# Deeptanshu-sankhwar/horizonml

Hardware: AMD Instinct MI355X
Metric: images/sec (higher is better)
Workload: dtype bf16; 1 GPU; model=resnet18_cifar10, global_batch=64, image=3x32x32, parallelism=dp1, optimizer=adam, exec=graph, comm=none

## Files before the change

### horizonml_amd/engine/flat.py

```python
from __future__ import annotations

from typing import List

import torch
import torch.nn as nn

from .. import ops as _ops
from ..models.layers import ConvBNAct, DepthwiseConvBNAct, Linear


SEG_CHUNK = 4096


class SegmentTable:

    def __init__(self, sizes, decay, adapt, device, chunk: int = SEG_CHUNK):
        sizes = [int(n) for n in sizes]
        if not sizes or min(sizes) < 1 or chunk < 1:
            raise ValueError("segments must be non-empty")
        if not len(sizes) == len(decay) == len(adapt):
            raise ValueError("one decay and one adapt flag per segment")
        if sum(sizes) >= 2 ** 31:
            raise ValueError("segment offsets are int32")
        chunks, meta, bounds = [], [], [0]
# ... 24 lines not shown
        self.lars, self.eta = bool(lars), float(eta)
        self.seg_mul = t.static_mul(self.wd)
        self.dynamic = self.max_norm > 0 or self.lars
        if self.dynamic:
            dev = mgr.master.device
            self.partials = torch.zeros(t.nchunks, 2, device=dev)
            self.seg_norms = torch.zeros(t.nseg, 2, device=dev)
            self.norm_out = torch.zeros(2, device=dev)

    def reduce(self, ext, mgr, grad_bf16, grad_scale):
        if self.dynamic:
            ext.seg_norms(mgr.master, mgr.grad, self.table.chunks,
                          self.table.seg_meta, self.partials, self.seg_norms,
                          self.seg_mul, self.norm_out, self.wd, self.max_norm,
                          self.lars, self.eta, grad_bf16, grad_scale)

    def last_grad_norm(self) -> float:
        if not self.dynamic:
            raise RuntimeError("the gradient norm is only computed with "
                               "clip_grad_norm > 0 or lars")
        return float(self.norm_out[0].cpu())


def _seg_state(mgr, wd, no_decay_1d, max_norm, lars=False, eta=1e-3):
    if max_norm < 0 or eta <= 0:
        raise ValueError("clip_grad_norm must be >= 0 and lars_eta > 0")
    if not (no_decay_1d or max_norm > 0 or lars):
        return None
    return _SegState(mgr, wd, no_decay_1d, max_norm, lars, eta)


class FlatParamManager:
    def __init__(self, model: nn.Module, device: torch.device):
        self._seg_tables = {}
        _ops.extension().set_wgrad_defer(True)
        params = [p for p in model.parameters() if p.requires_grad]
        total = sum(p.numel() for p in params)
        self.params = params
        self.numel = total
        self.master = torch.zeros(total, device=device)
        self.grad = torch.zeros(total, device=device)
        self.shadow = torch.zeros(total, device=device, dtype=torch.bfloat16)
        self.slices = {}
        off = 0
        for p in params:
            n = p.numel()
            with torch.no_grad():
                self.master[off:off + n].copy_(p.data.flatten())
            p.data = self.master[off:off + n].view(p.shape)
            p.grad = self.grad[off:off + n].view(p.shape)
            self.slices[id(p)] = (off, n)
            off += n
        with torch.no_grad():
            self.shadow.copy_(self.master)

        convs = []
        for m in model.modules():
            if isinstance(m, (ConvBNAct, Linear, DepthwiseConvBNAct)):
                woff, wn = self.slices[id(m.weight)]
                m.weight_bf16 = self.shadow[woff:woff + wn].view(
                    m.weight.shape)
                m._managed = True
                if isinstance(m, ConvBNAct):
                    convs.append((m, woff, wn))
        stats_total = sum(2 * m.out_ch for m, _, _ in convs)
        self.stats_arena = torch.zeros(max(1, stats_total), device=device)
        soff = 0
        for m, _, _ in convs:
            m._stats_buf = self.stats_arena[soff:soff + 2 * m.out_ch]
            soff += 2 * m.out_ch

        self.meta = None
        self.max_elem = 1
        if _ops.extension().dgrad_krsc_enabled():
            self.rsck = torch.zeros(0, device=device, dtype=torch.bfloat16)
            for m, _, _ in convs:
                if hasattr(m, "_w_rsck"):
                    del m._w_rsck
            return
        rsck_total = sum(wn for _, _, wn in convs)
        self.rsck = torch.zeros(rsck_total, device=device,
                                dtype=torch.bfloat16)
        meta: List[List[int]] = []
        doff = 0
        self.max_elem = 1
        for m, woff, wn in convs:
            K, R, S, C = m.weight.shape
# ... 3 lines not shown
            self.max_elem = max(self.max_elem, wn)
        self.meta = (torch.tensor(meta, dtype=torch.int32, device=device)
                     if meta else None)
        self.refresh_rsck()

    def refresh_rsck(self):
        if self.meta is not None:
            _ops.extension().permute_krsc_rsck(self.shadow, self.rsck,
                                               self.meta, self.max_elem)

    def zero_grad(self):
        self.grad.zero_()

    def segment_table(self, no_decay_1d: bool = False) -> SegmentTable:
        key = bool(no_decay_1d)
        if key not in self._seg_tables:
            one_d = [p.ndim <= 1 for p in self.params]
            self._seg_tables[key] = SegmentTable(
                [p.numel() for p in self.params],
                [not (key and d) for d in one_d], [not d for d in one_d],
                self.master.device)
        return self._seg_tables[key]


def _sched_buffers(schedule, dev):
    if schedule is None:
        return None, None
    return schedule.table().to(dev), torch.zeros(1, device=dev)


class HorizonAdam:

    def __init__(self, mgr: FlatParamManager, lr: float = 1e-3,
                 betas=(0.9, 0.999), eps: float = 1e-8,
                 weight_decay: float = 0.0, schedule=None,
                 decoupled_wd: bool = False, no_decay_1d: bool = False,
                 clip_grad_norm: float = 0.0):
        self.mgr = mgr
        self.seg = _seg_state(mgr, weight_decay, no_decay_1d, clip_grad_norm)
        self.lr, self.betas, self.eps, self.wd = lr, betas, eps, weight_decay
        self.schedule, self.decoupled = schedule, bool(decoupled_wd)
        dev = mgr.master.device
        self.m = torch.zeros_like(mgr.master)
        self.v = torch.zeros_like(mgr.master)
        self.step_t = torch.zeros(1, device=dev)
        self.lr_table, self.lr_out = _sched_buffers(schedule, dev)

    def step(self, zero_grad: bool = True, grad_bf16=None,
             grad_scale: float = 1.0, probe=None):
        ext = _ops.extension()
        ext.flush_wgrad()
        p0, p1, p2 = probe if probe is not None else (None, None, None)
        if self.seg is not None:
            self.seg.reduce(ext, self.mgr, grad_bf16, grad_scale)
            ext.adam_step_seg(self.mgr.master, self.mgr.grad, self.m, self.v,
                              self.mgr.shadow, self.step_t, self.lr_table,
                              self.lr_out, self.lr, self.betas[0],
                              self.betas[1], self.eps, self.decoupled,
                              zero_grad, self.seg.table.chunks,
                              self.seg.seg_mul, self.mgr.stats_arena,
                              grad_bf16, grad_scale, p0, p1, p2)
        elif self.schedule is None and not self.decoupled:
            ext.adam_step(self.mgr.master, self.mgr.grad, self.m,
                          self.v, self.mgr.shadow, self.step_t,
                          self.lr, self.betas[0], self.betas[1],
                          self.eps, self.wd, zero_grad,
                          self.mgr.stats_arena, grad_bf16,
                          grad_scale, p0, p1, p2)
        else:
            ext.adam_step_sched(self.mgr.master, self.mgr.grad, self.m,
                                self.v, self.mgr.shadow, self.step_t,
                                self.lr_table, self.lr_out, self.lr,
                                self.betas[0], self.betas[1], self.eps,
                                self.wd, self.decoupled, zero_grad,
                                self.mgr.stats_arena, grad_bf16, grad_scale,
                                p0, p1, p2)
        self.mgr.refresh_rsck()

    def current_lr(self) -> float:
        if self.lr_out is None:
            return float(self.lr)
        return float(self.lr_out.cpu())

    def last_grad_norm(self) -> float:
        if self.seg is None:
            raise RuntimeError("the gradient norm is only computed with "
                               "clip_grad_norm > 0 or lars")
        return self.seg.last_grad_norm()

    def set_step(self, n: int):
        self.step_t.fill_(float(n))

    def state_dict(self):
        return {"kind": "horizon_adam", "lr": self.lr, "betas": self.betas,
                "eps": self.eps, "weight_decay": self.wd,
                "m": self.m.detach().cpu(), "v": self.v.detach().cpu(),
                "step_t": self.step_t.detach().cpu()}

    def load_state_dict(self, state):
        if state.get("kind") != "horizon_adam":
            raise ValueError("checkpoint optimizer state is not HorizonAdam")
        with torch.no_grad():
            self.m.copy_(state["m"].to(self.m.device))
            self.v.copy_(state["v"].to(self.v.device))
            self.step_t.copy_(state["step_t"].to(self.step_t.device))


class HorizonSGD:

    def __init__(self, mgr: FlatParamManager, lr: float = 0.1,
                 momentum: float = 0.9, weight_decay: float = 0.0,
                 schedule=None, nesterov: bool = False,
                 no_decay_1d: bool = False, clip_grad_norm: float = 0.0,
                 lars: bool = False, lars_eta: float = 1e-3):
        if nesterov and not momentum > 0:
            raise ValueError("nesterov needs momentum > 0")
        self.mgr = mgr
        self.seg = _seg_state(mgr, weight_decay, no_decay_1d, clip_grad_norm,
                              lars, lars_eta)
        self.lr, self.mu, self.wd = lr, momentum, weight_decay
        self.schedule, self.nesterov = schedule, bool(nesterov)
        self.mom = (torch.zeros_like(mgr.master) if momentum > 0 else None)
        dev = mgr.master.device
        self.lr_table, self.lr_out = _sched_buffers(schedule, dev)
        self.step_t = (torch.zeros(1, device=dev)
                       if schedule is not None else None)

    def step(self, zero_grad: bool = True, grad_bf16=None,
             grad_scale: float = 1.0, probe=None):
        ext = _ops.extension()
        ext.flush_wgrad()
        p0, p1, p2 = probe if probe is not None else (None, None, None)
        if self.seg is not None:
            self.seg.reduce(ext, self.mgr, grad_bf16, grad_scale)
            ext.sgd_step_seg(self.mgr.master, self.mgr.grad, self.mom,
                             self.mgr.shadow, self.step_t, self.lr_table,
                             self.lr_out, self.lr, self.mu, self.nesterov,
                             zero_grad, self.seg.table.chunks,
                             self.seg.seg_mul, grad_bf16, grad_scale,
                             p0, p1, p2)
        elif self.schedule is None and not self.nesterov:
            ext.sgd_step(self.mgr.master, self.mgr.grad, self.mom,
                         self.mgr.shadow, self.lr, self.mu, self.wd,
                         zero_grad, grad_bf16, grad_scale,
                         p0, p1, p2)
        else:
            ext.sgd_step_sched(self.mgr.master, self.mgr.grad, self.mom,
                               self.mgr.shadow, self.step_t, self.lr_table,
                               self.lr_out, self.lr, self.mu, self.wd,
                               self.nesterov, zero_grad, grad_bf16,
                               grad_scale, p0, p1, p2)
        self.mgr.stats_arena.zero_()
        self.mgr.refresh_rsck()

    def current_lr(self) -> float:
        if self.lr_out is None:
            return float(self.lr)
        return float(self.lr_out.cpu())

    def last_grad_norm(self) -> float:
        if self.seg is None:
            raise RuntimeError("the gradient norm is only computed with "
                               "clip_grad_norm > 0 or lars")
        return self.seg.last_grad_norm()

    def set_step(self, n: int):
        if self.step_t is not None:
            self.step_t.fill_(float(n))

    def state_dict(self):
        state = {"kind": "horizon_sgd", "lr": self.lr, "momentum": self.mu,
                 "weight_decay": self.wd,
                 "mom": (self.mom.detach().cpu()
                         if self.mom is not None else None)}
        if self.step_t is not None:
            state["step_t"] = self.step_t.detach().cpu()
        return state

    def load_state_dict(self, state):
        if state.get("kind") != "horizon_sgd":
            raise ValueError("checkpoint optimizer state is not HorizonSGD")
        if (state.get("mom") is None) != (self.mom is None):
            raise ValueError("momentum buffer mismatch with checkpoint")
        with torch.no_grad():
            if self.mom is not None:
                self.mom.copy_(state["mom"].to(self.mom.device))
            if self.step_t is not None and state.get("step_t") is not None:
                self.step_t.copy_(state["step_t"].to(self.step_t.device))
```

### horizonml_amd/ops/csrc/bind.cpp

```cpp
#include <torch/extension.h>
#include <c10/hip/HIPStream.h>
#include <c10/hip/HIPCachingAllocator.h>

#include <memory>
#include <vector>

#include "launch.h"

namespace {

using torch::Tensor;

hipStream_t cur_stream() { return c10::hip::getCurrentHIPStream().stream(); }

bool g_deterministic = false;
void set_deterministic(bool on) {
  g_deterministic = on;
  set_kernels_deterministic(on ? 1 : 0);
}
bool deterministic_enabled() { return g_deterministic; }

void set_bn_owner(bool on) { set_kernels_bn_owner(on ? 1 : 0); }
bool bn_owner_enabled() { return kernels_bn_owner() != 0; }
std::vector<int64_t> bn_owner_launches() {
  long f = 0, b = 0;
  bn_owner_launch_counts(&f, &b);
  return {(int64_t)f, (int64_t)b};
// ... 9 lines not shown

bool g_tap_clip = env_long("HZ_TAP_CLIP", 1) != 0;
void set_tap_clip(bool on) { g_tap_clip = on; }
bool tap_clip_enabled() { return g_tap_clip; }

std::vector<int64_t> conv_tap_window(int64_t H, int64_t W, int64_t R,
                                     int64_t S, int64_t stride, int64_t pad) {
  TORCH_CHECK(stride >= 1 && pad >= 0 && R >= 1 && S >= 1 &&
                  H + 2 * pad >= R && W + 2 * pad >= S,
              "conv_tap_window: empty output or bad geometry");
  ConvP p{};
  p.H = (int)H;
  p.W = (int)W;
  p.C = 1;
  p.R = p.Rf = (int)R;
  p.S = p.Sf = (int)S;
  p.str = (int)stride;
  p.pad = (int)pad;
  p.Ho = (p.H + 2 * p.pad - p.R) / p.str + 1;
  p.Wo = (p.W + 2 * p.pad - p.S) / p.str + 1;
  p = clip_taps(p);
  return {p.r0, p.s0, p.R, p.S};
}

struct PendingWgrad {
  torch::Tensor x, dconv, dw;
  ConvP p;
};

bool g_wgrad_defer = false;
std::vector<PendingWgrad> g_pending;
torch::Tensor g_wgrad_ws;

void set_wgrad_defer(bool on) { g_wgrad_defer = on; }
bool wgrad_defer_enabled() { return g_wgrad_defer; }
int64_t wgrad_pending() { return (int64_t)g_pending.size(); }

static inline int cdiv_i(long a, long b) { return (int)((a + b - 1) / b); }

void flush_one_group(int lo, int hi);

void flush_wgrad() {
  if (g_pending.empty()) return;
  const int total = (int)g_pending.size();
  int lo = 0;
  while (lo < total) {
// ... 403 lines not shown
  if (has_res) {
    dres = empty_cl_bf16(p.Nb, K, p.Ho, p.Wo, x);
    dres_ptr = dres.data_ptr();
  }
  if (own)
    launch_bn_bwd_owner(dy.data_ptr(), y.data_ptr(), convout.data_ptr(),
                        save_mean.data_ptr<float>(),
                        save_invstd.data_ptr<float>(),
                        gamma.data_ptr<float>(), beta.data_ptr<float>(),
                        sum_dz.data_ptr<float>(), sum_dzx.data_ptr<float>(),
                        dconv.data_ptr(), dres_ptr, (long)p.M, K, mask_mode,
                        own, st);
  else
    launch_bn_bwd_apply(dy.data_ptr(), y.data_ptr(), convout.data_ptr(),
                        save_mean.data_ptr<float>(),
                        save_invstd.data_ptr<float>(),
                        gamma.data_ptr<float>(), beta.data_ptr<float>(),
                        sum_dz.data_ptr<float>(), sum_dzx.data_ptr<float>(),
                        dconv.data_ptr(), dres_ptr, (long)p.M, K, mask_mode,
                        st);

  Tensor dw = direct ? *dw_out
                     : at::zeros({(int64_t)K, R, S, (int64_t)p.C}, fopt);
  if (direct && g_wgrad_defer) {
    g_pending.push_back({x, dconv, dw, p});
  } else {
    int msplit = wgrad_msplit(p);
    Tensor ws;
    float* ws_ptr = nullptr;
    if (msplit > 1) {
      ws = at::empty({(long)msplit * K * p.Kd}, fopt);
      ws_ptr = ws.data_ptr<float>();
    }
    launch_wgrad(x.data_ptr(), dconv.data_ptr(), dw.data_ptr<float>(), ws_ptr,
                 p, (int)g_wgrad_tr, st);
  }

  TORCH_CHECK(need_dx || !fuse_up.has_value(),
              "fuse_up requires need_dx (the fused reduce rides the dx "
              "production)");
  Tensor dx;
  if (need_dx)
    dx = dgrad_dx(dconv, w, w_rsck, p, dx_accum, fuse_up, (int)up_mask_mode,
                  st);
  return {dx, dw, sum_dzx, sum_dz, dres};
}
// ... 535 lines not shown
                  c10::optional<Tensor> probe_sumsq,
                  c10::optional<Tensor> probe_out) {
  check_f32(master, "master");
  check_probe(probe_prev, probe_sumsq, probe_out);
  TORCH_CHECK(grad.numel() == master.numel()
                  && (!mom.has_value() || mom->numel() == master.numel()),
              "grad / mom must match master's size");
  TORCH_CHECK(!nesterov || (mom.has_value() && mu > 0.0),
              "nesterov needs a momentum buffer and momentum > 0");
  SegTable t = seg_table(chunks, seg_mul, master);
  long T = 0;
  const float* table = sched_table(lr_table, master, &T);
  TORCH_CHECK(table == nullptr || step_t.has_value(),
              "lr_table needs the step_t device counter");
  float* out = sched_scalar(lr_out, master, "lr_out");
  float* st = sched_scalar(step_t, master, "step_t");
  launch_sgd_step_seg(master.data_ptr<float>(), grad.data_ptr<float>(),
                      opt_ptr<float>(mom), opt_ptr(shadow), (float)lr,
                      (float)mu, zero_grad ? 1 : 0, opt_ptr(grad_bf16),
                      (float)grad_scale, opt_ptr<float>(probe_prev),
                      opt_ptr<float>(probe_sumsq), opt_ptr<float>(probe_out),
                      st, table, T, out, nesterov ? 1 : 0, t.chunks,
                      t.nchunks, t.seg_mul, cur_stream());
}

void permute_krsc_rsck(Tensor src, Tensor dst, Tensor meta,
                       int64_t max_elem) {
  TORCH_CHECK(meta.scalar_type() == torch::kInt32 && meta.is_cuda());
  launch_permute_krsc_rsck(src.data_ptr(), dst.data_ptr(),
                           meta.data_ptr<int>(), (int)meta.size(0),
                           (int)max_elem, cur_stream());
}

void grad_divergence(Tensor g, Tensor prev, Tensor sumsq, Tensor out,
                     bool skip_first) {
  launch_grad_divergence(g.data_ptr<float>(), prev.data_ptr<float>(),
                         sumsq.data_ptr<float>(), out.data_ptr<float>(),
                         g.numel(), skip_first ? 1 : 0, cur_stream());
}

void bn_reduce_bench(Tensor dy, Tensor y, Tensor x, Tensor mean,
                     Tensor invstd, Tensor gamma, Tensor beta, Tensor sdz,
                     Tensor sdzx, int64_t M, int64_t C, int64_t mask) {
  launch_bnact_bwd_reduce(dy.data_ptr(), y.data_ptr(), x.data_ptr(),
                          mean.data_ptr<float>(), invstd.data_ptr<float>(),
                          gamma.data_ptr<float>(), beta.data_ptr<float>(),
// ... 154 lines not shown
        py::arg("probe_out") = py::none());
  m.def("seg_norms", &seg_norms, py::arg("master"), py::arg("grad"),
        py::arg("chunks"), py::arg("seg_meta"), py::arg("partials"),
        py::arg("seg_norms"), py::arg("seg_mul"), py::arg("norm_out"),
        py::arg("wd"), py::arg("max_norm"), py::arg("lars"), py::arg("eta"),
        py::arg("grad_bf16") = py::none(), py::arg("grad_scale") = 1.0);
  m.def("adam_step_seg", &adam_step_seg, py::arg("master"), py::arg("grad"),
        py::arg("m"), py::arg("v"), py::arg("shadow"), py::arg("step_t"),
        py::arg("lr_table"), py::arg("lr_out"), py::arg("lr"), py::arg("b1"),
        py::arg("b2"), py::arg("eps"), py::arg("decoupled"),
        py::arg("zero_grad"), py::arg("chunks"), py::arg("seg_mul"),
        py::arg("extra_zero") = py::none(), py::arg("grad_bf16") = py::none(),
        py::arg("grad_scale") = 1.0, py::arg("probe_prev") = py::none(),
        py::arg("probe_sumsq") = py::none(),
        py::arg("probe_out") = py::none());
  m.def("sgd_step_seg", &sgd_step_seg, py::arg("master"), py::arg("grad"),
        py::arg("mom"), py::arg("shadow"), py::arg("step_t"),
        py::arg("lr_table"), py::arg("lr_out"), py::arg("lr"), py::arg("mu"),
        py::arg("nesterov"), py::arg("zero_grad"), py::arg("chunks"),
        py::arg("seg_mul"), py::arg("grad_bf16") = py::none(),
        py::arg("grad_scale") = 1.0, py::arg("probe_prev") = py::none(),
        py::arg("probe_sumsq") = py::none(),
        py::arg("probe_out") = py::none());
  m.def("permute_krsc_rsck", &permute_krsc_rsck);
  m.def("grad_divergence", &grad_divergence);
  m.def("normalize_u8", &normalize_u8);
  m.def("augment_normalize_u8", &augment_normalize_u8, py::arg("x"),
        py::arg("state"), py::arg("mean"), py::arg("std"), py::arg("pad"),
        py::arg("flip"), py::arg("params") = py::none());
  m.def("bn_reduce_bench", &bn_reduce_bench);
  m.def("bn_fwd_pair_bench", &bn_fwd_pair_bench);
  m.def("bn_bwd_pair_bench", &bn_bwd_pair_bench);
  m.def("set_bn_owner", &set_bn_owner);
  m.def("bn_owner_enabled", &bn_owner_enabled);
  m.def("bn_owner_launches", &bn_owner_launches);
  m.def("set_deterministic", &set_deterministic);
  m.def("deterministic_enabled", &deterministic_enabled);
  m.def("set_wgrad_defer", &set_wgrad_defer);
  m.def("wgrad_defer_enabled", &wgrad_defer_enabled);
  m.def("wgrad_pending", &wgrad_pending);
  m.def("flush_wgrad", &flush_wgrad);
  m.def("flush_wgrad_range", &flush_wgrad_range);
  m.def("wgrad_only", &wgrad_only);
  m.def("conv_dgrad_only", &conv_dgrad_only);
  m.def("set_dgrad_krsc", &set_dgrad_krsc);
  m.def("dgrad_krsc_enabled", &dgrad_krsc_enabled);
// ... 7 lines not shown
```

### horizonml_amd/ops/csrc/elem_kernels.hip

```cpp
#include <cstdio>

#include "common.h"

union F8 {
  float4 q[2];
  float f[8];
};

DEV F8 load_f8(const float* p) {
  F8 v;
  v.q[0] = *(const float4*)p;
  v.q[1] = *(const float4*)(p + 4);
  return v;
}

template <bool F32SRC, int ACT, bool TRAIN>
__global__ __launch_bounds__(256) void k_bn_apply(
    const void* __restrict__ xv, const bf16* __restrict__ res,
    bf16* __restrict__ y, bf16* __restrict__ convout,
    const float* __restrict__ stats,
    const float* __restrict__ gamma, const float* __restrict__ beta,
    float* __restrict__ running_mean, float* __restrict__ running_var,
    float* __restrict__ save_mean, float* __restrict__ save_invstd,
    long M, int C, float momentum, float eps, int nsplit) {
// ... 1499 lines not shown
    const float* __restrict__ logits, const long* __restrict__ target,
    float* __restrict__ loss, float* __restrict__ dlogits, int B, int NC) {
  ce_body<false>(logits, target, loss, dlogits, B, NC, 0.f,
                 blockIdx.x * blockDim.x + threadIdx.x,
                 gridDim.x * blockDim.x);
}

__global__ __launch_bounds__(256) void k_ce_ls_fwd_bwd_det(
    const float* __restrict__ logits, const long* __restrict__ target,
    float* __restrict__ loss, float* __restrict__ dlogits, int B, int NC,
    float eps) {
  ce_det_body<true>(logits, target, loss, dlogits, B, NC, eps);
}

__global__ __launch_bounds__(256) void k_ce_ls_fwd_bwd(
    const float* __restrict__ logits, const long* __restrict__ target,
    float* __restrict__ loss, float* __restrict__ dlogits, int B, int NC,
    float eps) {
  ce_body<true>(logits, target, loss, dlogits, B, NC, eps,
                blockIdx.x * blockDim.x + threadIdx.x,
                gridDim.x * blockDim.x);
}

template <bool DECOUPLED, bool SEG = false>
__device__ __forceinline__ void adam_body(
    float* __restrict__ master, float* __restrict__ grad,
    float* __restrict__ m, float* __restrict__ v, bf16* __restrict__ shadow,
    const float* __restrict__ step_t, long n, float lr, float b1, float b2,
    float eps, float wd, int zero_grad, float* __restrict__ extra_zero,
    long n_extra, const bf16* __restrict__ gsrc, float gscale,
    float* __restrict__ prev, float* __restrict__ sumsq, long i0,
    long istride, float gmul = 1.f) {
  for (long i = i0; i < n_extra; i += istride) extra_zero[i] = 0.f;
  float t = step_t[0];
  float bc1 = 1.f - __powf(b1, t), bc2 = 1.f - __powf(b2, t);
  float acc = 0.f;
  for (long i = i0; i < n; i += istride) {
    float gl = grad[i];
    float g = gsrc != nullptr ? b2f(gsrc[i]) * gscale : gl;
    if (prev != nullptr) {
      float d = gl - prev[i];
      prev[i] = gl;
      acc += d * d;
    }
    if (SEG && gmul != 1.f) g *= gmul;
    float w = master[i];
    if (DECOUPLED) {
      if (wd != 0.f) w *= 1.f - lr * wd;
    } else {
      if (wd != 0.f) g += wd * w;
    }
    float mi = b1 * m[i] + (1.f - b1) * g;
    float vi = b2 * v[i] + (1.f - b2) * g * g;
    m[i] = mi;
    v[i] = vi;
    w -= lr * (mi / bc1) / (sqrtf(vi / bc2) + eps);
    master[i] = w;
    if (shadow != nullptr) shadow[i] = f2b(w);
    if (zero_grad) grad[i] = 0.f;
  }
  if (prev != nullptr) {
    acc = wave_reduce_sum(acc);
    __shared__ float ws[4];
    if ((threadIdx.x & 63) == 0) ws[threadIdx.x >> 6] = acc;
    __syncthreads();
    if (threadIdx.x == 0)
      atomicAdd(sumsq, ws[0] + ws[1] + ws[2] + ws[3]);
  }
}

template <bool NESTEROV, bool SEG = false>
__device__ __forceinline__ void sgd_body(
    float* __restrict__ master, float* __restrict__ grad,
    float* __restrict__ mom, bf16* __restrict__ shadow, long n, float lr,
    float mu, float wd, int zero_grad, const bf16* __restrict__ gsrc,
    float gscale, float* __restrict__ prev, float* __restrict__ sumsq,
    long i0, long istride, float gmul = 1.f) {
  float acc = 0.f;
  for (long i = i0; i < n; i += istride) {
    float gl = grad[i];
    float g = gsrc != nullptr ? b2f(gsrc[i]) * gscale : gl;
    if (prev != nullptr) {
      float d = gl - prev[i];
      prev[i] = gl;
      acc += d * d;
    }
    if (SEG && gmul != 1.f) g *= gmul;
    float w = master[i];
    if (wd != 0.f) g += wd * w;
    float u = (mom != nullptr) ? (mu * mom[i] + g) : g;
    if (mom != nullptr) mom[i] = u;
    if (NESTEROV)
      w -= lr * (g + mu * u);
    else
      w -= lr * u;
    master[i] = w;
    if (shadow != nullptr) shadow[i] = f2b(w);
    if (zero_grad) grad[i] = 0.f;
  }
  if (prev != nullptr) {
    acc = wave_reduce_sum(acc);
    __shared__ float ws[4];
// ... 229 lines not shown
__global__ __launch_bounds__(256) void k_adam_step_seg(
    float* __restrict__ master, float* __restrict__ grad,
    float* __restrict__ m, float* __restrict__ v, bf16* __restrict__ shadow,
    const float* __restrict__ step_t, float lr, float b1, float b2,
    float eps, int zero_grad, float* __restrict__ extra_zero, long n_extra,
    const bf16* __restrict__ gsrc, float gscale, float* __restrict__ prev,
    float* __restrict__ sumsq, const float* __restrict__ lr_table, long T,
    float* __restrict__ lr_out, const int* __restrict__ chunks,
    const float* __restrict__ seg_mul) {
  lr = sched_lr(step_t, lr_table, T, lr, lr_out);
  for (long i = (long)blockIdx.x * 256 + threadIdx.x; i < n_extra;
       i += (long)gridDim.x * 256)
    extra_zero[i] = 0.f;
  const int c = blockIdx.x;
  const int s = chunks[c * 3];
  const long start = chunks[c * 3 + 1];
  const long end = start + chunks[c * 3 + 2];
  adam_body<DECOUPLED, true>(master, grad, m, v, shadow, step_t, end, lr, b1,
                             b2, eps, seg_mul[2 * s + 1], zero_grad, nullptr,
                             0, gsrc, gscale, prev, sumsq,
                             start + threadIdx.x, 256, seg_mul[2 * s]);
}

__global__ __launch_bounds__(256) void k_permute_krsc_rsck(
    const bf16* __restrict__ src, bf16* __restrict__ dst,
    const int* __restrict__ meta, int nconv) {
  __shared__ bf16 tile[32][33];
  const int ci = blockIdx.y;
  if (ci >= nconv) return;
  const int soff = meta[ci * 4 + 0], doff = meta[ci * 4 + 1];
  const int nelem = meta[ci * 4 + 2];
  const int K = meta[ci * 4 + 3] >> 16, C = meta[ci * 4 + 3] & 0xffff;
  const int RS = nelem / (K * C);
  const int ktiles = (K + 31) / 32, ctiles = (C + 31) / 32;
  const int tiles_per_rs = ktiles * ctiles;
  const int total_tiles = RS * tiles_per_rs;
  const int tc = threadIdx.x & 31, tr = threadIdx.x >> 5;
  for (int t = blockIdx.x; t < total_tiles; t += gridDim.x) {
    int rs = t / tiles_per_rs, rem = t % tiles_per_rs;
    int k0 = (rem / ctiles) * 32, c0 = (rem % ctiles) * 32;
    const bf16* s = src + soff + (long)rs * C;
#pragma unroll
    for (int i = 0; i < 4; i++) {
      int ko = k0 + tr + i * 8, c = c0 + tc;
      tile[tr + i * 8][tc] = (ko < K && c < C)
          ? s[(long)ko * RS * C + c] : (bf16)0.f;
// ... 666 lines not shown
  if (decoupled) LA(true); else LA(false);
#undef LA
  if (prev != nullptr)
    k_gdiv_finalize<<<1, 1, 0, st>>>(sumsq, divout, 0);
}

void launch_sgd_step_seg(float* master, float* grad, float* mom, void* shadow,
                         float lr, float mu, int zero_grad, const void* gsrc,
                         float gscale, float* prev, float* sumsq,
                         float* divout, float* step_t, const float* lr_table,
                         long T, float* lr_out, int nesterov,
                         const int* chunks, int nchunks, const float* seg_mul,
                         hipStream_t st) {
  if (lr_table != nullptr) k_inc_step<<<1, 1, 0, st>>>(step_t);
#define LS(N) k_sgd_step_seg<N><<<nchunks, 256, 0, st>>>( \
    master, grad, mom, (bf16*)shadow, lr, mu, zero_grad, (const bf16*)gsrc, \
    gscale, prev, sumsq, step_t, lr_table, T, lr_out, chunks, seg_mul)
  if (nesterov) LS(true); else LS(false);
#undef LS
  if (prev != nullptr)
    k_gdiv_finalize<<<1, 1, 0, st>>>(sumsq, divout, 0);
}

void launch_permute_krsc_rsck(const void* src, void* dst, const int* meta,
                              int nconv, int max_elem, hipStream_t st) {
  dim3 grid(gsz((long)max_elem, 1024), nconv);
  k_permute_krsc_rsck<<<grid, 256, 0, st>>>((const bf16*)src, (bf16*)dst,
                                            meta, nconv);
}

void launch_grad_divergence(const float* g, float* prev, float* sumsq,
                            float* out, long n, int skip_first,
                            hipStream_t st) {
  k_gdiv_partial<<<gsz(n >> 2), 256, 0, st>>>(g, prev, sumsq, n);
  k_gdiv_finalize<<<1, 1, 0, st>>>(sumsq, out, skip_first);
}

void launch_normalize_u8(const void* x, void* y, long total, int C, long HW,
                         float mean, float std, hipStream_t st) {
  k_normalize_u8<<<gsz(total), 256, 0, st>>>((const unsigned char*)x,
                                             (bf16*)y, total, C, HW, mean,
                                             std);
}

void launch_augment_normalize_u8(const void* x, void* y, void* state,
                                 const int* params, long N, int C, int H,
// ... 17 lines not shown
```

### horizonml_amd/ops/csrc/launch.h

```cpp
#pragma once
#include <hip/hip_runtime_api.h>

#include <cstdlib>
#include <type_traits>

struct ConvP {
  int Nb, H, W, C, K;
  int Ho, Wo, R, S;
  int str, pad;
  int M, Kd;
  int r0, s0, Rf, Sf;
};

struct MagicP {
  unsigned m[4];
  int s[4];
  unsigned d[4];
};

constexpr int WG_MAX_TASKS = 20;

struct WgradTask {
  const void* X;
  const void* Dz;
// ... 81 lines not shown
        last = r;
        break;
      }
    }
  *lo = last < 0 ? 0 : first;
  *n = last < 0 ? 0 : last - first + 1;
}

inline ConvP clip_taps(ConvP p) {
  int r0, rn, s0, sn;
  tap_range(p.H, p.Ho, p.Rf, p.str, p.pad, &r0, &rn);
  tap_range(p.W, p.Wo, p.Sf, p.str, p.pad, &s0, &sn);
  if (rn <= 0 || sn <= 0) return p;
  p.r0 = r0;
  p.s0 = s0;
  p.R = rn;
  p.S = sn;
  p.Kd = rn * sn * p.C;
  return p;
}

inline bool taps_clipped(const ConvP& p) {
  return p.R != p.Rf || p.S != p.Sf;
}

inline long env_long(const char* name, long dflt) {
  const char* e = getenv(name);
  return e ? atol(e) : dflt;
}

extern "C" {

int conv_fwd_splitk(ConvP p);
int conv_dgrad_splitk(ConvP p);
void launch_conv_fwd(const void* x, const void* w, void* y, float* stats,
                     ConvP p, hipStream_t st);
void launch_conv_fwd_splitk(const void* x, const void* w, float* ws, ConvP p,
                            int splitk, hipStream_t st);
void launch_conv_dgrad(const void* dz, const void* w, void* dx, float* ws,
                       int splitk, ConvP p, int accum, int w_layout,
                       hipStream_t st);
void launch_gemm_bf16(const void* a, const void* b, void* c, int M, int N,
                      int K, hipStream_t st);
int wgrad_msplit(ConvP p);
void launch_wgrad(const void* x, const void* dz, float* dw, float* ws,
                  ConvP p, int tr, hipStream_t st);
// ... 110 lines not shown
                        const float* lr_table, long T, float* lr_out,
                        int nesterov, hipStream_t st);
void launch_seg_norms(const float* master, const float* grad,
                      const void* gsrc, float gscale, const int* chunks,
                      int nchunks, const int* seg_meta, int nseg,
                      float* partials, float* seg_norms, float* seg_mul,
                      float* norm_out, float wd, float max_norm, int lars,
                      float eta, hipStream_t st);
void launch_adam_step_seg(float* master, float* grad, float* m, float* v,
                          void* shadow, float* step_t, float lr, float b1,
                          float b2, float eps, int zero_grad,
                          float* extra_zero, long n_extra, const void* gsrc,
                          float gscale, float* prev, float* sumsq,
                          float* divout, const float* lr_table, long T,
                          float* lr_out, int decoupled, const int* chunks,
                          int nchunks, const float* seg_mul, hipStream_t st);
void launch_sgd_step_seg(float* master, float* grad, float* mom, void* shadow,
                         float lr, float mu, int zero_grad, const void* gsrc,
                         float gscale, float* prev, float* sumsq,
                         float* divout, float* step_t, const float* lr_table,
                         long T, float* lr_out, int nesterov,
                         const int* chunks, int nchunks, const float* seg_mul,
                         hipStream_t st);

void launch_permute_krsc_rsck(const void* src, void* dst, const int* meta,
                              int nconv, int max_elem, hipStream_t st);
void launch_grad_divergence(const float* g, float* prev, float* sumsq,
                            float* out, long n, int skip_first,
                            hipStream_t st);
void launch_normalize_u8(const void* x, void* y, long total, int C, long HW,
                         float mean, float std, hipStream_t st);
void launch_augment_normalize_u8(const void* x, void* y, void* state,
                                 const int* params, long N, int C, int H,
                                 int W, int pad, int flip, float mean,
                                 float std, hipStream_t st);

}
```

Baseline: 71560 images/sec.

## Skip optimizer updates on structurally dead conv filter taps via a live-chunk table

Records, per weight-gradient buffer, the range of filter taps that can ever receive gradient given the conv geometry. From that it builds a strided chunk table covering only live weight elements. New Adam and SGD kernels walk this table, so the optimizer skips weights whose gradient is structurally zero. Buffers with nonzero values in dead taps are demoted to full updates. The cost is host-side table building, registry bookkeeping and strided access. The table is not built during graph capture.

```diff
diff --git a/horizonml_amd/engine/flat.py b/horizonml_amd/engine/flat.py
--- a/horizonml_amd/engine/flat.py
+++ b/horizonml_amd/engine/flat.py
@@ -70,6 +70,77 @@
         return float(self.norm_out[0].cpu())
 
 
+LIVE_CHUNK = 4096
+
+
+def build_live_chunks(numel, windows, chunk: int = LIVE_CHUNK):
+    numel, chunk = int(numel), int(chunk)
+    if numel < 1 or numel >= 2 ** 31 or chunk < 1:
+        raise ValueError("live table offsets are int32")
+    spans, families, cursor, n_dead = [], [], 0, 0
+    for off, K, Rf, Sf, C, r0, R, s0, S in sorted(
+            tuple(int(x) for x in w) for w in windows):
+        kdf = Rf * Sf * C
+        if min(K, Rf, Sf, C, R, S) < 1 or min(r0, s0) < 0 \
+                or r0 + R > Rf or s0 + S > Sf:
+            raise ValueError("tap window outside its filter")
+        if off < cursor or off + K * kdf > numel:
+            raise ValueError("conv weights overlap or leave the buffer")
+        if R == Rf and S == Sf:
+            continue
+        if off > cursor:
+            spans.append((cursor, off))
+        cursor = off + K * kdf
+        n_dead += K * (Rf * Sf - R * S) * C
+        if S == Sf:
+            families.append((off + r0 * Sf * C, R * Sf * C, kdf, K))
+        else:
+            families += [(off + ((r0 + r) * Sf + s0) * C, S * C, kdf, K)
+                         for r in range(R)]
+    if cursor < numel:
+        spans.append((cursor, numel))
+
+    chunks = []
+
+    def cut(lo, hi):
+        chunks.extend((o, min(chunk, hi - o), 0, 1)
+                      for o in range(lo, hi, chunk))
+
+    for lo, hi in spans:
+        cut(lo, hi)
+    for start, run_len, pitch, nruns in families:
+        if run_len >= chunk or nruns == 1:
+            for r in range(nruns):
+                cut(start + r * pitch, start + r * pitch + run_len)
+            continue
+        group = chunk // run_len
+        chunks.extend((start + r * pitch, run_len, pitch,
+                       min(group, nruns - r))
+                      for r in range(0, nruns, group))
+    for start, run_len, pitch, nruns in chunks:
+        if not (run_len >= 1 and nruns >= 1 and run_len * nruns <= chunk
+                and start >= 0 and pitch >= 0
+                and (nruns == 1 or pitch >= run_len)
+                and start + (nruns - 1) * pitch + run_len <= numel):
+            raise AssertionError("live chunk out of bounds")
+    return chunks, n_dead
+
+
+class _LiveTable:
+
+    def __init__(self):
+        self.version = -1
+        self.bufs = []
+        self.chunks = None
+        self.n_dead = 0
+        self.n_demoted = 0
+        self.nchunks = 0
+
+    def covers(self, bufs):
+        have = {t.data_ptr() for t in self.bufs}
+        return all(t.data_ptr() in have for t in bufs)
+
+
 def _seg_state(mgr, wd, no_decay_1d, max_norm, lars=False, eta=1e-3):
     if max_norm < 0 or eta <= 0:
         raise ValueError("clip_grad_norm must be >= 0 and lars_eta > 0")
@@ -88,6 +159,8 @@
         self.numel = total
         self.master = torch.zeros(total, device=device)
         self.grad = torch.zeros(total, device=device)
+        _ops.extension().tap_window_reset(
+            self.grad.data_ptr(), self.grad.data_ptr() + 4 * total)
         self.shadow = torch.zeros(total, device=device, dtype=torch.bfloat16)
         self.slices = {}
         off = 0
@@ -111,6 +184,9 @@
                 m._managed = True
                 if isinstance(m, ConvBNAct):
                     convs.append((m, woff, wn))
+        self._conv_shapes = {woff: tuple(m.weight.shape)
+                             for m, woff, _ in convs}
+        self._live = _LiveTable()
         stats_total = sum(2 * m.out_ch for m, _, _ in convs)
         self.stats_arena = torch.zeros(max(1, stats_total), device=device)
         soff = 0
@@ -160,6 +236,72 @@
                 self.master.device)
         return self._seg_tables[key]
 
+    def live_windows(self):
+        base, out = self.grad.data_ptr(), []
+        for ptr, K, Rf, Sf, C, r0, R, s0, S in \
+                _ops.extension().tap_window_registry():
+            off, rem = divmod(ptr - base, 4)
+            if rem == 0 and self._conv_shapes.get(off) == (K, Rf, Sf, C):
+                out.append((off, K, Rf, Sf, C, r0, R, s0, S))
+        return sorted(out)
+
+    def invalidate_live_table(self):
+        self._live.version = -1
+
+    def live_table_info(self):
+        lt = self._live
+        state = ("unbuilt" if lt.version < 0
+                 else "none" if lt.chunks is None else "live")
+        return {"state": state, "version": lt.version,
+                "skipped": lt.n_dead if state == "live" else 0,
+                "nchunks": lt.nchunks if state == "live" else 0,
+                "demoted": lt.n_demoted}
+
+    def live_chunks(self, bufs):
+        ext = _ops.extension()
+        if not ext.opt_skip_dead_enabled():
+            return None
+        lt = self._live
+        bufs = [t for t in bufs if t is not None]
+        version = ext.tap_window_version()
+        if lt.version != version or not lt.covers(bufs):
+            if torch.cuda.is_current_stream_capturing():
+                return None
+            have = {t.data_ptr() for t in bufs}
+            bufs += [t for t in lt.bufs if t.data_ptr() not in have]
+            self._build_live_table(version, bufs)
+        return lt.chunks
+
+    def _build_live_table(self, version, bufs):
+        lt = self._live
+        wins = self.live_windows()
+        clipped = [w for w in wins if w[6] * w[8] < w[2] * w[3]]
+        lt.n_demoted = 0
+        if clipped:
+            counts = []
+            for off, K, Rf, Sf, C, r0, R, s0, S in clipped:
+                n, c = K * Rf * Sf * C, 0
+                for t in [self.grad] + bufs:
+                    bits = t[off:off + n].view(
+                        torch.int32 if t.element_size() == 4 else torch.int16
+                    ).view(K, Rf, Sf, C)
+                    c = c + torch.count_nonzero(bits) - torch.count_nonzero(
+                        bits[:, r0:r0 + R, s0:s0 + S])
+                counts.append(c)
+            bad = torch.stack(counts).cpu().tolist()
+            lt.n_demoted = sum(1 for b in bad if b)
+            clipped = [w for w, b in zip(clipped, bad) if not b]
+        chunks, lt.n_dead = build_live_chunks(self.numel, clipped)
+        if lt.n_dead:
+            lt.chunks = torch.tensor(chunks, dtype=torch.int32,
+                                     device=self.master.device)
+            lt.nchunks = len(chunks)
+            with torch.no_grad():
+                self.shadow.copy_(self.master)
+        else:
+            lt.chunks, lt.nchunks = None, 0
+        lt.version, lt.bufs = version, bufs
+
 
 def _sched_buffers(schedule, dev):
     if schedule is None:
@@ -183,12 +325,16 @@
         self.v = torch.zeros_like(mgr.master)
         self.step_t = torch.zeros(1, device=dev)
         self.lr_table, self.lr_out = _sched_buffers(schedule, dev)
+        self._live_stale = False
 
     def step(self, zero_grad: bool = True, grad_bf16=None,
              grad_scale: float = 1.0, probe=None):
         ext = _ops.extension()
         ext.flush_wgrad()
         p0, p1, p2 = probe if probe is not None else (None, None, None)
+        if self._live_stale:
+            self.mgr.invalidate_live_table()
+            self._live_stale = False
         if self.seg is not None:
             self.seg.reduce(ext, self.mgr, grad_bf16, grad_scale)
             ext.adam_step_seg(self.mgr.master, self.mgr.grad, self.m, self.v,
@@ -198,6 +344,14 @@
                               zero_grad, self.seg.table.chunks,
                               self.seg.seg_mul, self.mgr.stats_arena,
                               grad_bf16, grad_scale, p0, p1, p2)
+        elif self.wd == 0 and (live := self.mgr.live_chunks(
+                (self.m, self.v, p0, grad_bf16))) is not None:
+            ext.adam_step_live(self.mgr.master, self.mgr.grad, self.m,
+                               self.v, self.mgr.shadow, self.step_t,
+                               self.lr_table, self.lr_out, self.lr,
+                               self.betas[0], self.betas[1], self.eps,
+                               zero_grad, live, self.mgr.stats_arena,
+                               grad_bf16, grad_scale, p0, p1, p2)
         elif self.schedule is None and not self.decoupled:
             ext.adam_step(self.mgr.master, self.mgr.grad, self.m,
                           self.v, self.mgr.shadow, self.step_t,
@@ -238,6 +392,7 @@
     def load_state_dict(self, state):
         if state.get("kind") != "horizon_adam":
             raise ValueError("checkpoint optimizer state is not HorizonAdam")
+        self._live_stale = True
         with torch.no_grad():
             self.m.copy_(state["m"].to(self.m.device))
             self.v.copy_(state["v"].to(self.v.device))
@@ -263,12 +418,16 @@
         self.lr_table, self.lr_out = _sched_buffers(schedule, dev)
         self.step_t = (torch.zeros(1, device=dev)
                        if schedule is not None else None)
+        self._live_stale = False
 
     def step(self, zero_grad: bool = True, grad_bf16=None,
              grad_scale: float = 1.0, probe=None):
         ext = _ops.extension()
         ext.flush_wgrad()
         p0, p1, p2 = probe if probe is not None else (None, None, None)
+        if self._live_stale:
+            self.mgr.invalidate_live_table()
+            self._live_stale = False
         if self.seg is not None:
             self.seg.reduce(ext, self.mgr, grad_bf16, grad_scale)
             ext.sgd_step_seg(self.mgr.master, self.mgr.grad, self.mom,
@@ -277,6 +436,13 @@
                              zero_grad, self.seg.table.chunks,
                              self.seg.seg_mul, grad_bf16, grad_scale,
                              p0, p1, p2)
+        elif self.wd == 0 and (live := self.mgr.live_chunks(
+                (self.mom, p0, grad_bf16))) is not None:
+            ext.sgd_step_live(self.mgr.master, self.mgr.grad, self.mom,
+                              self.mgr.shadow, self.step_t, self.lr_table,
+                              self.lr_out, self.lr, self.mu, self.nesterov,
+                              zero_grad, live, grad_bf16, grad_scale,
+                              p0, p1, p2)
         elif self.schedule is None and not self.nesterov:
             ext.sgd_step(self.mgr.master, self.mgr.grad, self.mom,
                          self.mgr.shadow, self.lr, self.mu, self.wd,
@@ -320,6 +486,7 @@
             raise ValueError("checkpoint optimizer state is not HorizonSGD")
         if (state.get("mom") is None) != (self.mom is None):
             raise ValueError("momentum buffer mismatch with checkpoint")
+        self._live_stale = True
         with torch.no_grad():
             if self.mom is not None:
                 self.mom.copy_(state["mom"].to(self.mom.device))
diff --git a/horizonml_amd/ops/csrc/bind.cpp b/horizonml_amd/ops/csrc/bind.cpp
--- a/horizonml_amd/ops/csrc/bind.cpp
+++ b/horizonml_amd/ops/csrc/bind.cpp
@@ -2,7 +2,10 @@
 #include <c10/hip/HIPStream.h>
 #include <c10/hip/HIPCachingAllocator.h>
 
+#include <algorithm>
 #include <memory>
+#include <mutex>
+#include <unordered_map>
 #include <vector>
 
 #include "launch.h"
@@ -58,6 +61,73 @@
   p = clip_taps(p);
   return {p.r0, p.s0, p.R, p.S};
 }
+
+struct TapWindow {
+  int K, Rf, Sf, C;
+  int r0, R, s0, S;
+};
+std::mutex g_tapwin_mu;
+std::unordered_map<uintptr_t, TapWindow> g_tapwin;
+int64_t g_tapwin_version = 0;
+
+void record_tap_window(const Tensor& dw, const ConvP& p) {
+  const ConvP g = geometric_taps(p);
+  const uintptr_t key = (uintptr_t)dw.data_ptr();
+  std::lock_guard<std::mutex> lock(g_tapwin_mu);
+  auto it = g_tapwin.find(key);
+  if (it == g_tapwin.end() || it->second.K != g.K || it->second.Rf != g.Rf ||
+      it->second.Sf != g.Sf || it->second.C != g.C) {
+    g_tapwin[key] = {g.K, g.Rf, g.Sf, g.C, g.r0, g.R, g.s0, g.S};
+    g_tapwin_version++;
+    return;
+  }
+  TapWindow& w = it->second;
+  const int r0 = std::min(w.r0, g.r0), s0 = std::min(w.s0, g.s0);
+  const int r1 = std::max(w.r0 + w.R, g.r0 + g.R);
+  const int s1 = std::max(w.s0 + w.S, g.s0 + g.S);
+  if (r0 != w.r0 || s0 != w.s0 || r1 - r0 != w.R || s1 - s0 != w.S) {
+    w.r0 = r0;
+    w.R = r1 - r0;
+    w.s0 = s0;
+    w.S = s1 - s0;
+    g_tapwin_version++;
+  }
+}
+
+std::vector<std::vector<int64_t>> tap_window_registry() {
+  std::lock_guard<std::mutex> lock(g_tapwin_mu);
+  std::vector<std::vector<int64_t>> out;
+  out.reserve(g_tapwin.size());
+  for (const auto& kv : g_tapwin) {
+    const TapWindow& w = kv.second;
+    out.push_back({(int64_t)kv.first, w.K, w.Rf, w.Sf, w.C, w.r0, w.R, w.s0,
+                   w.S});
+  }
+  return out;
+}
+
+int64_t tap_window_version() {
+  std::lock_guard<std::mutex> lock(g_tapwin_mu);
+  return g_tapwin_version;
+}
+
+void tap_window_reset(int64_t lo, int64_t hi) {
+  std::lock_guard<std::mutex> lock(g_tapwin_mu);
+  if (hi <= lo) {
+    g_tapwin.clear();
+  } else {
+    for (auto it = g_tapwin.begin(); it != g_tapwin.end();)
+      if (it->first >= (uintptr_t)lo && it->first < (uintptr_t)hi)
+        it = g_tapwin.erase(it);
+      else
+        ++it;
+  }
+  g_tapwin_version++;
+}
+
+bool g_opt_skip_dead = env_long("HZ_OPT_SKIP_DEAD", 1) != 0;
+void set_opt_skip_dead(bool on) { g_opt_skip_dead = on; }
+bool opt_skip_dead_enabled() { return g_opt_skip_dead; }
 
 struct PendingWgrad {
   torch::Tensor x, dconv, dw;
@@ -507,6 +577,7 @@
 
   Tensor dw = direct ? *dw_out
                      : at::zeros({(int64_t)K, R, S, (int64_t)p.C}, fopt);
+  if (direct) record_tap_window(dw, p);
   if (direct && g_wgrad_defer) {
     g_pending.push_back({x, dconv, dw, p});
   } else {
@@ -1088,6 +1159,86 @@
                       opt_ptr<float>(probe_sumsq), opt_ptr<float>(probe_out),
                       st, table, T, out, nesterov ? 1 : 0, t.chunks,
                       t.nchunks, t.seg_mul, cur_stream());
+}
+
+const int* live_table(const Tensor& live, const Tensor& master,
+                      int* nchunks) {
+  TORCH_CHECK(live.scalar_type() == torch::kInt32 && live.dim() == 2
+                  && live.size(1) == 4 && live.size(0) >= 1
+                  && live.is_contiguous()
+                  && live.device() == master.device()
+                  && (uintptr_t)live.data_ptr() % 16 == 0,
+              "live must be a contiguous, 16-byte aligned int32 [nchunks,4] "
+              "tensor on master's device");
+  *nchunks = (int)live.size(0);
+  return live.data_ptr<int>();
+}
+
+void adam_step_live(Tensor master, Tensor grad, Tensor m, Tensor v,
+                    c10::optional<Tensor> shadow, Tensor step_t,
+                    c10::optional<Tensor> lr_table,
+                    c10::optional<Tensor> lr_out, double lr, double b1,
+                    double b2, double eps, bool zero_grad, Tensor live,
+                    c10::optional<Tensor> extra_zero,
+                    c10::optional<Tensor> grad_bf16, double grad_scale,
+                    c10::optional<Tensor> probe_prev,
+                    c10::optional<Tensor> probe_sumsq,
+                    c10::optional<Tensor> probe_out) {
+  check_f32(master, "master");
+  check_probe(probe_prev, probe_sumsq, probe_out);
+  TORCH_CHECK(grad.numel() == master.numel() && m.numel() == master.numel()
+                  && v.numel() == master.numel(),
+              "grad / m / v must match master's size");
+  int nchunks = 0;
+  const int* chunks = live_table(live, master, &nchunks);
+  long T = 0;
+  const float* table = sched_table(lr_table, master, &T);
+  float* out = sched_scalar(lr_out, master, "lr_out");
+  float* st = sched_scalar(step_t, master, "step_t");
+  launch_adam_step_live(master.data_ptr<float>(), grad.data_ptr<float>(),
+                        m.data_ptr<float>(), v.data_ptr<float>(),
+                        opt_ptr(shadow), st, (float)lr, (float)b1, (float)b2,
+                        (float)eps, zero_grad ? 1 : 0,
+                        opt_ptr<float>(extra_zero),
+                        extra_zero.has_value() ? extra_zero->numel() : 0,
+                        opt_ptr(grad_bf16), (float)grad_scale,
+                        opt_ptr<float>(probe_prev),
+                        opt_ptr<float>(probe_sumsq),
+                        opt_ptr<float>(probe_out), table, T, out, chunks,
+                        nchunks, cur_stream());
+}
+
+void sgd_step_live(Tensor master, Tensor grad, c10::optional<Tensor> mom,
+                   c10::optional<Tensor> shadow, c10::optional<Tensor> step_t,
+                   c10::optional<Tensor> lr_table,
+                   c10::optional<Tensor> lr_out, double lr, double mu,
+                   bool nesterov, bool zero_grad, Tensor live,
+                   c10::optional<Tensor> grad_bf16, double grad_scale,
+                   c10::optional<Tensor> probe_prev,
+                   c10::optional<Tensor> probe_sumsq,
+                   c10::optional<Tensor> probe_out) {
+  check_f32(master, "master");
+  check_probe(probe_prev, probe_sumsq, probe_out);
+  TORCH_CHECK(grad.numel() == master.numel()
+                  && (!mom.has_value() || mom->numel() == master.numel()),
+              "grad / mom must match master's size");
+  TORCH_CHECK(!nesterov || (mom.has_value() && mu > 0.0),
+              "nesterov needs a momentum buffer and momentum > 0");
+  int nchunks = 0;
+  const int* chunks = live_table(live, master, &nchunks);
+  long T = 0;
+  const float* table = sched_table(lr_table, master, &T);
+  TORCH_CHECK(table == nullptr || step_t.has_value(),
+              "lr_table needs the step_t device counter");
+  float* out = sched_scalar(lr_out, master, "lr_out");
+  float* st = sched_scalar(step_t, master, "step_t");
+  launch_sgd_step_live(master.data_ptr<float>(), grad.data_ptr<float>(),
+                       opt_ptr<float>(mom), opt_ptr(shadow), (float)lr,
+                       (float)mu, zero_grad ? 1 : 0, opt_ptr(grad_bf16),
+                       (float)grad_scale, opt_ptr<float>(probe_prev),
+                       opt_ptr<float>(probe_sumsq), opt_ptr<float>(probe_out),
+                       st, table, T, out, nesterov ? 1 : 0, chunks, nchunks,
+                       cur_stream());
 }
 
 void permute_krsc_rsck(Tensor src, Tensor dst, Tensor meta,
@@ -1288,6 +1439,29 @@
         py::arg("grad_scale") = 1.0, py::arg("probe_prev") = py::none(),
         py::arg("probe_sumsq") = py::none(),
         py::arg("probe_out") = py::none());
+  m.def("adam_step_live", &adam_step_live, py::arg("master"),
+        py::arg("grad"), py::arg("m"), py::arg("v"), py::arg("shadow"),
+        py::arg("step_t"), py::arg("lr_table"), py::arg("lr_out"),
+        py::arg("lr"), py::arg("b1"), py::arg("b2"), py::arg("eps"),
+        py::arg("zero_grad"), py::arg("live"),
+        py::arg("extra_zero") = py::none(), py::arg("grad_bf16") = py::none(),
+        py::arg("grad_scale") = 1.0, py::arg("probe_prev") = py::none(),
+        py::arg("probe_sumsq") = py::none(),
+        py::arg("probe_out") = py::none());
+  m.def("sgd_step_live", &sgd_step_live, py::arg("master"), py::arg("grad"),
+        py::arg("mom"), py::arg("shadow"), py::arg("step_t"),
+        py::arg("lr_table"), py::arg("lr_out"), py::arg("lr"), py::arg("mu"),
+        py::arg("nesterov"), py::arg("zero_grad"), py::arg("live"),
+        py::arg("grad_bf16") = py::none(), py::arg("grad_scale") = 1.0,
+        py::arg("probe_prev") = py::none(),
+        py::arg("probe_sumsq") = py::none(),
+        py::arg("probe_out") = py::none());
+  m.def("tap_window_registry", &tap_window_registry);
+  m.def("tap_window_version", &tap_window_version);
+  m.def("tap_window_reset", &tap_window_reset, py::arg("lo") = 0,
+        py::arg("hi") = 0);
+  m.def("set_opt_skip_dead", &set_opt_skip_dead);
+  m.def("opt_skip_dead_enabled", &opt_skip_dead_enabled);
   m.def("permute_krsc_rsck", &permute_krsc_rsck);
   m.def("grad_divergence", &grad_divergence);
   m.def("normalize_u8", &normalize_u8);
diff --git a/horizonml_amd/ops/csrc/elem_kernels.hip b/horizonml_amd/ops/csrc/elem_kernels.hip
--- a/horizonml_amd/ops/csrc/elem_kernels.hip
+++ b/horizonml_amd/ops/csrc/elem_kernels.hip
@@ -1545,7 +1545,28 @@
                 gridDim.x * blockDim.x);
 }
 
-template <bool DECOUPLED, bool SEG = false>
+struct LiveIdx {
+  unsigned r, j, dq, dm, run_len;
+  long base, pitch;
+  __device__ __forceinline__ LiveIdx(long i0, long istride, unsigned run_len_,
+                                     long base_, long pitch_)
+      : run_len(run_len_), base(base_), pitch(pitch_) {
+    r = (unsigned)i0 / run_len;
+    j = (unsigned)i0 - r * run_len;
+    dq = (unsigned)istride / run_len;
+    dm = (unsigned)istride - dq * run_len;
+  }
+  __device__ __forceinline__ long at() const {
+    return base + (long)r * pitch + j;
+  }
+  __device__ __forceinline__ void next() {
+    r += dq;
+    j += dm;
+    if (j >= run_len) { j -= run_len; r++; }
+  }
+};
+
+template <bool DECOUPLED, bool SEG = false, bool LIVE = false>
 __device__ __forceinline__ void adam_body(
     float* __restrict__ master, float* __restrict__ grad,
     float* __restrict__ m, float* __restrict__ v, bf16* __restrict__ shadow,
@@ -1553,12 +1574,16 @@
     float eps, float wd, int zero_grad, float* __restrict__ extra_zero,
     long n_extra, const bf16* __restrict__ gsrc, float gscale,
     float* __restrict__ prev, float* __restrict__ sumsq, long i0,
-    long istride, float gmul = 1.f) {
+    long istride, float gmul = 1.f, unsigned run_len = 1, long base = 0,
+    long run_pitch = 0) {
   for (long i = i0; i < n_extra; i += istride) extra_zero[i] = 0.f;
   float t = step_t[0];
   float bc1 = 1.f - __powf(b1, t), bc2 = 1.f - __powf(b2, t);
   float acc = 0.f;
-  for (long i = i0; i < n; i += istride) {
+  LiveIdx li(LIVE ? i0 : 0, LIVE ? istride : 0, run_len, base, run_pitch);
+  for (long e = i0; e < n; e += istride) {
+    const long i = LIVE ? li.at() : e;
+    if (LIVE) li.next();
     float gl = grad[i];
     float g = gsrc != nullptr ? b2f(gsrc[i]) * gscale : gl;
     if (prev != nullptr) {
@@ -1592,15 +1617,19 @@
   }
 }
 
-template <bool NESTEROV, bool SEG = false>
+template <bool NESTEROV, bool SEG = false, bool LIVE = false>
 __device__ __forceinline__ void sgd_body(
     float* __restrict__ master, float* __restrict__ grad,
     float* __restrict__ mom, bf16* __restrict__ shadow, long n, float lr,
     float mu, float wd, int zero_grad, const bf16* __restrict__ gsrc,
     float gscale, float* __restrict__ prev, float* __restrict__ sumsq,
-    long i0, long istride, float gmul = 1.f) {
+    long i0, long istride, float gmul = 1.f, unsigned run_len = 1,
+    long base = 0, long run_pitch = 0) {
   float acc = 0.f;
-  for (long i = i0; i < n; i += istride) {
+  LiveIdx li(LIVE ? i0 : 0, LIVE ? istride : 0, run_len, base, run_pitch);
+  for (long e = i0; e < n; e += istride) {
+    const long i = LIVE ? li.at() : e;
+    if (LIVE) li.next();
     float gl = grad[i];
     float g = gsrc != nullptr ? b2f(gsrc[i]) * gscale : gl;
     if (prev != nullptr) {
@@ -1876,6 +1905,42 @@
                              start + threadIdx.x, 256, seg_mul[2 * s]);
 }
 
+__global__ __launch_bounds__(256) void k_adam_step_live(
+    float* __restrict__ master, float* __restrict__ grad,
+    float* __restrict__ m, float* __restrict__ v, bf16* __restrict__ shadow,
+    const float* __restrict__ step_t, float lr, float b1, float b2,
+    float eps, int zero_grad, float* __restrict__ extra_zero, long n_extra,
+    const bf16* __restrict__ gsrc, float gscale, float* __restrict__ prev,
+    float* __restrict__ sumsq, const float* __restrict__ lr_table, long T,
+    float* __restrict__ lr_out, const int4* __restrict__ live) {
+  lr = sched_lr(step_t, lr_table, T, lr, lr_out);
+  for (long i = (long)blockIdx.x * 256 + threadIdx.x; i < n_extra;
+       i += (long)gridDim.x * 256)
+    extra_zero[i] = 0.f;
+  const int4 c = live[blockIdx.x];
+  adam_body<false, false, true>(master, grad, m, v, shadow, step_t,
+                                (long)c.w * c.y, lr, b1, b2, eps, 0.f,
+                                zero_grad, nullptr, 0, gsrc, gscale, prev,
+                                sumsq, threadIdx.x, 256, 1.f, (unsigned)c.y,
+                                c.x, c.z);
+}
+
+template <bool NESTEROV>
+__global__ __launch_bounds__(256) void k_sgd_step_live(
+    float* __restrict__ master, float* __restrict__ grad,
+    float* __restrict__ mom, bf16* __restrict__ shadow, float lr, float mu,
+    int zero_grad, const bf16* __restrict__ gsrc, float gscale,
+    float* __restrict__ prev, float* __restrict__ sumsq,
+    const float* __restrict__ step_t, const float* __restrict__ lr_table,
+    long T, float* __restrict__ lr_out, const int4* __restrict__ live) {
+  lr = sched_lr(step_t, lr_table, T, lr, lr_out);
+  const int4 c = live[blockIdx.x];
+  sgd_body<NESTEROV, false, true>(master, grad, mom, shadow, (long)c.w * c.y,
+                                  lr, mu, 0.f, zero_grad, gsrc, gscale, prev,
+                                  sumsq, threadIdx.x, 256, 1.f,
+                                  (unsigned)c.y, c.x, c.z);
+}
+
 __global__ __launch_bounds__(256) void k_permute_krsc_rsck(
     const bf16* __restrict__ src, bf16* __restrict__ dst,
     const int* __restrict__ meta, int nconv) {
@@ -2588,6 +2653,40 @@
     k_gdiv_finalize<<<1, 1, 0, st>>>(sumsq, divout, 0);
 }
 
+void launch_adam_step_live(float* master, float* grad, float* m, float* v,
+                           void* shadow, float* step_t, float lr, float b1,
+                           float b2, float eps, int zero_grad,
+                           float* extra_zero, long n_extra, const void* gsrc,
+                           float gscale, float* prev, float* sumsq,
+                           float* divout, const float* lr_table, long T,
+                           float* lr_out, const int* live, int nchunks,
+                           hipStream_t st) {
+  k_inc_step<<<1, 1, 0, st>>>(step_t);
+  k_adam_step_live<<<nchunks, 256, 0, st>>>(
+      master, grad, m, v, (bf16*)shadow, step_t, lr, b1, b2, eps, zero_grad,
+      extra_zero, n_extra, (const bf16*)gsrc, gscale, prev, sumsq, lr_table,
+      T, lr_out, (const int4*)live);
+  if (prev != nullptr)
+    k_gdiv_finalize<<<1, 1, 0, st>>>(sumsq, divout, 0);
+}
+
+void launch_sgd_step_live(float* master, float* grad, float* mom,
+                          void* shadow, float lr, float mu, int zero_grad,
+                          const void* gsrc, float gscale, float* prev,
+                          float* sumsq, float* divout, float* step_t,
+                          const float* lr_table, long T, float* lr_out,
+                          int nesterov, const int* live, int nchunks,
+                          hipStream_t st) {
+  if (lr_table != nullptr) k_inc_step<<<1, 1, 0, st>>>(step_t);
+#define LS(N) k_sgd_step_live<N><<<nchunks, 256, 0, st>>>( \
+    master, grad, mom, (bf16*)shadow, lr, mu, zero_grad, (const bf16*)gsrc, \
+    gscale, prev, sumsq, step_t, lr_table, T, lr_out, (const int4*)live)
+  if (nesterov) LS(true); else LS(false);
+#undef LS
+  if (prev != nullptr)
+    k_gdiv_finalize<<<1, 1, 0, st>>>(sumsq, divout, 0);
+}
+
 void launch_permute_krsc_rsck(const void* src, void* dst, const int* meta,
                               int nconv, int max_elem, hipStream_t st) {
   dim3 grid(gsz((long)max_elem, 1024), nconv);
diff --git a/horizonml_amd/ops/csrc/launch.h b/horizonml_amd/ops/csrc/launch.h
--- a/horizonml_amd/ops/csrc/launch.h
+++ b/horizonml_amd/ops/csrc/launch.h
@@ -127,6 +127,14 @@
 
 inline bool taps_clipped(const ConvP& p) {
   return p.R != p.Rf || p.S != p.Sf;
+}
+
+inline ConvP geometric_taps(ConvP p) {
+  p.r0 = p.s0 = 0;
+  p.R = p.Rf;
+  p.S = p.Sf;
+  p.Kd = p.Rf * p.Sf * p.C;
+  return clip_taps(p);
 }
 
 inline long env_long(const char* name, long dflt) {
@@ -283,6 +291,21 @@
                          long T, float* lr_out, int nesterov,
                          const int* chunks, int nchunks, const float* seg_mul,
                          hipStream_t st);
+void launch_adam_step_live(float* master, float* grad, float* m, float* v,
+                           void* shadow, float* step_t, float lr, float b1,
+                           float b2, float eps, int zero_grad,
+                           float* extra_zero, long n_extra, const void* gsrc,
+                           float gscale, float* prev, float* sumsq,
+                           float* divout, const float* lr_table, long T,
+                           float* lr_out, const int* live, int nchunks,
+                           hipStream_t st);
+void launch_sgd_step_live(float* master, float* grad, float* mom,
+                          void* shadow, float lr, float mu, int zero_grad,
+                          const void* gsrc, float gscale, float* prev,
+                          float* sumsq, float* divout, float* step_t,
+                          const float* lr_table, long T, float* lr_out,
+                          int nesterov, const int* live, int nchunks,
+                          hipStream_t st);
 
 void launch_permute_krsc_rsck(const void* src, void* dst, const int* meta,
                               int nconv, int max_elem, hipStream_t st);
```

Result: faster. 75660 images/sec, median of 6 (+5.7%).
